# brech1/keaki

Measured on AMD Instinct MI355X. Metric: BN254 G1 scalar-mults/sec on 2^24-point MSM (per GPU), higher is better.
Workload: dtype u32 limbs, 256-bit Montgomery modular integer (9 x 29-bit lazy limbs in the bucket kernel, 8 x 32 elsewhere)

## Files before the change

keaki_amd/csrc/msm.hip.h:

```cpp
#pragma once
#include <type_traits>
#include "bn254_curve.hip.h"
#include "fq29.hip.h"
#include "xyzz29.hip.h"
#include "jac29.hip.h"
#include "xyzz29_g2.hip.h"

namespace bn254 {

typedef uint16_t u16;
typedef u32 v4u_t __attribute__((ext_vector_type(4)));
constexpr u32 DIGIT_NONE = 0xFFFFFFFFu;
#ifndef STAMP
#define STAMP(cond, i) do { } while (0)
#endif

struct MsmShape {
  u32 n;
  u32 c;
  u32 W;
  u32 k;
  u32 stride;
};
KDEV u32 msm_width(const MsmShape& s, u32 w) { return w < s.k ? s.c : s.c - 1; }
KDEV u32 msm_bit_offset(const MsmShape& s, u32 w) { return w < s.k ? w * s.c : s.k * s.c + (w - s.k) * (s.c - 1); }
KDEV u32 msm_nbuckets(const MsmShape& s, u32 w) { u32 wd = msm_width(s, w); return w == s.W - 1 ? (1u << wd) : (1u << (wd - 1)); }
KDEV u32 msm_bucket_base(const MsmShape& s, u32 w) {
  return w <= s.k ? w * (1u << (s.c - 1)) : s.k * (1u << (s.c - 1)) + (w - s.k) * (1u << (s.c - 2));
}
struct MsmPlan {
  MsmShape s;
  size_t nb;
  u32 max_b;
};
inline MsmPlan msm_make_plan(size_t n, int c_target) {
  MsmPlan p;
  u32 W = (254 + c_target - 1) / c_target;
  u32 base = 254 / W, rem = 254 % W;
  p.s.n = (u32)n;
  p.s.W = W;
  p.s.stride = 0;
  if (rem == 0) { p.s.c = base; p.s.k = W; } else { p.s.c = base + 1; p.s.k = rem; }
  size_t nb = 0; u32 mb = 0;
  for (u32 w = 0; w < W; w++) {
    u32 wd = w < p.s.k ? p.s.c : p.s.c - 1;
    u32 b = (w == W - 1) ? (1u << wd) : (1u << (wd - 1));
    nb += b; if (b > mb) mb = b;
  }
  p.nb = nb; p.max_b = mb;
  return p;
}

template <class Emit>
KDEV void msm_for_each_digit_canon(const u32 (&canon)[8], const MsmShape& s, Emit emit) {
  u32 v[8];
#pragma unroll
  for (int j = 0; j < 8; j++) v[j] = canon[j];
  u32 carry = 0;
  for (u32 w = 0; w < s.W; w++) {
    const u32 wd = msm_width(s, w);
    const u32 full = 1u << wd, half = full >> 1;
    u32 coef = (v[0] & (full - 1u)) + carry;
#pragma unroll
    for (int j = 0; j < 7; j++) v[j] = (u32)((((u64)v[j + 1] << 32) | v[j]) >> wd);
    v[7] >>= wd;
    if (w == s.W - 1) {
      if (coef) emit(w, coef - 1u);
    } else if (coef > half) {
      carry = 1;
      if (coef != full) emit(w, (full - coef - 1u) | 0x80000000u);
    } else {
      carry = 0;
      if (coef) emit(w, coef - 1u);
    }
  }
}

template <u32 W> struct StaticPlan {
  static constexpr u32 base = 254 / W, rem = 254 % W;
  static constexpr u32 c = rem ? base + 1 : base, k = rem ? rem : W;
  static constexpr u32 width(u32 w) { return w < k ? c : c - 1; }
  static constexpr u32 offset(u32 w) { return w < k ? w * c : k * c + (w - k) * (c - 1); }
};
template <u32 W>
KDEV void msm_digits_static(const u32 (&v)[8], u32 (&code)[W]) {
  typedef StaticPlan<W> P;
  u32 carry = 0;
#pragma unroll
  for (u32 w = 0; w < W; w++) {
    const u32 off = P::offset(w), wd = P::width(w), j = off >> 5, sh = off & 31;
    const u32 lo = v[j], hi = j + 1 < 8 ? v[j + 1] : 0u;
    const u32 d = (sh + wd <= 32 ? lo >> sh : __builtin_amdgcn_alignbit(hi, lo, sh)) & ((1u << wd) - 1u);
    const u32 full = 1u << wd, half = full >> 1;
    const u32 coef = d + carry;
    if (w == W - 1) {
      code[w] = coef ? coef - 1u : DIGIT_NONE;
    } else {
      const bool neg = coef > half;
      carry = neg ? 1u : 0u;
      code[w] = neg ? (coef != full ? ((full - coef - 1u) | 0x80000000u) : DIGIT_NONE) : (coef ? coef - 1u : DIGIT_NONE);
    }
  }
}

template <class Emit>
KDEV void msm_for_each_digit(const Fr& k, const MsmShape& s, Emit emit) {
  u32 v[8];
  fp_from_mont<FrParams>(v, k);
  msm_for_each_digit_canon(v, s, emit);
}

constexpr u32 T1_THREADS = 1024;
constexpr u32 T1_PER = 3;
constexpr u32 T1_CAP = 36864;
constexpr u32 PART_MAX_BINS = 2048;
constexpr u32 C2_THREADS = 1024;
constexpr u32 C2_CAP = 32768;
constexpr u32 PART_MAX_FINE_SHIFT = 11;
constexpr u32 PART_MAX_FINE = 1u << PART_MAX_FINE_SHIFT;
constexpr u32 SEG_INLINE = 4;
constexpr u32 TE_WPOS = 12, TE_SIGN = 19, TE_FINE = 20, TE_VALID = 0x80000000u;

struct PartShape {
  u32 nbins, lb;
  u32 shift, hb;
  u32 nf;
  u32 tile;
  u32 ntiles;
  u32 te;
  u32 geom;
};
KDEV u32 part_bin(const PartShape& ps, u32 g) { return (g >> ps.shift) & (ps.nbins - 1u); }
KDEV u32 part_fine(const PartShape& ps, u32 g) { return ((g >> (ps.shift + ps.lb)) << ps.shift) | (g & ((1u << ps.shift) - 1u)); }
KDEV u32 part_bucket(const PartShape& ps, u32 bin, u32 f) { return ((f >> ps.shift) << (ps.shift + ps.lb)) | (bin << ps.shift) | (f & ((1u << ps.shift) - 1u)); }
inline bool part_make_shape(size_t n, u32 W, size_t nb, PartShape* ps, int lb_override = -1, int hb_override = -1, int geom_override = -1) {
  u32 lg = 0;
  while (((size_t)1 << lg) < nb) lg++;
  const size_t pairs = n * (size_t)W;
  const u32 lb_max = pairs > ((size_t)C2_CAP << 13) ? 11u : 10u;
  u32 lb = 0;
  while (lb < lb_max && ((size_t)C2_CAP << lb) < pairs) lb++;
  if (lb_override >= 0 && lb_override <= 11) lb = (u32)lb_override;
  if (lb > lg) lb = lg;
  if (lg - lb > PART_MAX_FINE_SHIFT) lb = lg - PART_MAX_FINE_SHIFT;
  if (lb > 11) return false;
  const u32 fb = lg - lb;
  ps->lb = lb; ps->nbins = 1u << lb;
  ps->hb = fb < 3 ? fb : 3u;
  if (hb_override >= 0 && (u32)hb_override <= fb) ps->hb = (u32)hb_override;
  ps->shift = fb - ps->hb;
  ps->nf = 1u << fb;
  u32 tile = W ? T1_CAP / W : T1_THREADS * T1_PER;
  if (tile > T1_THREADS * T1_PER) tile = T1_THREADS * T1_PER;
  if (tile == 0 || W >= (1u << (TE_SIGN - TE_WPOS))) return false;
  ps->tile = tile;
  ps->ntiles = (u32)((n + tile - 1) / tile);
  ps->te = tile * W;
  const u32 mean = ps->te / ps->nbins;
  ps->geom = mean <= 24 ? 0u : mean <= 48 ? 1u : mean <= 100 ? 2u : 3u;
  if (geom_override >= 0) ps->geom = (u32)geom_override;
  return true;
}
inline size_t part_max_chunks(size_t pairs, u32 nbins) { return pairs / C2_CAP + nbins + 1; }

__device__ __forceinline__ void lds_barrier() { asm volatile("s_waitcnt lgkmcnt(0)\n\ts_barrier" ::: "memory"); }

__device__ __forceinline__ u32 lds_exclusive_scan4(u32* a, u32 len, u32* wsum) {
  const u32 t = threadIdx.x, lane = t & 63, wid = t >> 6, nw = blockDim.x >> 6;
  lds_barrier();
  u32 x[4], sum = 0;
#pragma unroll
  for (u32 i = 0; i < 4; i++) { x[i] = 4 * t + i < len ? a[4 * t + i] : 0u; sum += x[i]; }
  u32 v = sum;
#pragma unroll
  for (int o = 1; o < 64; o <<= 1) { u32 y = __shfl_up(v, o, 64); if (lane >= (u32)o) v += y; }
  if (lane == 63) wsum[wid] = v;
  lds_barrier();
  u32 base = 0, tot = 0;
  for (u32 k = 0; k < nw; k++) { u32 sv = wsum[k]; if (k < wid) base += sv; tot += sv; }
  u32 ex = base + v - sum;
#pragma unroll
  for (u32 i = 0; i < 4; i++) { if (4 * t + i < len) a[4 * t + i] = ex; ex += x[i]; }
  lds_barrier();
  return tot;
}

template <u32 WS>
static __global__ void __launch_bounds__(T1_THREADS) k_tile_sort(const Fr* __restrict__ scalars, MsmShape s, PartShape ps, u32* __restrict__ tiles,
                                                                 u16* __restrict__ tstart) {
  __shared__ u32 ent[T1_CAP + 64];
  __shared__ u32 cur[PART_MAX_BINS + 64];
  __shared__ u32 wsum[T1_THREADS / 64];
  constexpr u32 NC = WS ? WS : 1u;
  Fr nxt[T1_PER];
  auto request = [&](u32 tile, u32 tl) {
#pragma unroll
    for (u32 p = 0; p < T1_PER; p++) {
      const u32 li = p * T1_THREADS + tl;
      const size_t i = (size_t)tile * ps.tile + li;
      nxt[p] = scalars[li < ps.tile && i < s.n ? i : (size_t)s.n - 1];
    }
  };
  if (blockIdx.x < ps.ntiles) request(blockIdx.x, threadIdx.x);
  for (u32 tile = blockIdx.x; tile < ps.ntiles; tile += gridDim.x) {
    u32 t = threadIdx.x;
    asm volatile("" : "+v"(t));
    [[maybe_unused]] const u32 sk = (tile - blockIdx.x) / gridDim.x;
    STAMP(blockIdx.x == 100 && t == 0 && sk < 4, 2048 + sk * 16 + 0);
    u32 canon[T1_PER][8];
    bool act[T1_PER];
#pragma unroll
    for (u32 p = 0; p < T1_PER; p++) {
      const u32 li = p * T1_THREADS + t;
      act[p] = li < ps.tile && (size_t)tile * ps.tile + li < s.n;
      fp_from_mont<FrParams>(canon[p], nxt[p]);
    }
    if (tile + gridDim.x < ps.ntiles) request(tile + gridDim.x, t);
    STAMP(blockIdx.x == 100 && t == 0 && sk < 4, 2048 + sk * 16 + 1);
    for (u32 b = t; b < ps.nbins; b += T1_THREADS) cur[b] = 0;
    if (t < 64) cur[PART_MAX_BINS + t] = 0;
    lds_barrier();
    STAMP(blockIdx.x == 100 && t == 0 && sk < 4, 2048 + sk * 16 + 2);
#pragma unroll
    for (u32 p = 0; p < T1_PER; p++) {
      if constexpr (WS != 0) {
        u32 code[NC];
        msm_digits_static<NC>(canon[p], code);
#pragma unroll
        for (u32 w = 0; w < NC; w++) {
          const u32 g = (s.stride ? 0u : msm_bucket_base(s, w)) + (code[w] & 0x7FFFFFFFu);
          atomicAdd(&cur[act[p] && code[w] != DIGIT_NONE ? part_bin(ps, g) : PART_MAX_BINS + (t & 63u)], 1u);
        }
      } else if (act[p]) {
        msm_for_each_digit_canon(canon[p], s, [&](u32 w, u32 cd) {
          const u32 g = (s.stride ? 0u : msm_bucket_base(s, w)) + (cd & 0x7FFFFFFFu);
          atomicAdd(&cur[part_bin(ps, g)], 1u);
        });
      }
    }
    STAMP(blockIdx.x == 100 && t == 0 && sk < 4, 2048 + sk * 16 + 3);
    const u32 m = lds_exclusive_scan4(cur, ps.nbins, wsum);
    u16* ts = tstart + (size_t)tile * (ps.nbins + 1);
    for (u32 b = t; b < ps.nbins; b += T1_THREADS) ts[b] = (u16)cur[b];
    if (t == 0) ts[ps.nbins] = (u16)m;
    lds_barrier();
    STAMP(blockIdx.x == 100 && t == 0 && sk < 4, 2048 + sk * 16 + 4);
#pragma unroll
    for (u32 p = 0; p < T1_PER; p++)
#pragma unroll
      for (u32 j = 0; j < 8; j++) asm volatile("" : "+v"(canon[p][j]));
#pragma unroll
    for (u32 p = 0; p < T1_PER; p++) {
      const u32 li = p * T1_THREADS + t;
      if constexpr (WS != 0) {
        u32 code[NC];
        msm_digits_static<NC>(canon[p], code);
#pragma unroll
        for (u32 w = 0; w < NC; w++) {
          const u32 cd = code[w];
          const bool ok = act[p] && cd != DIGIT_NONE;
          const u32 g = (s.stride ? 0u : msm_bucket_base(s, w)) + (cd & 0x7FFFFFFFu);
          const u32 pos = atomicAdd(&cur[ok ? part_bin(ps, g) : PART_MAX_BINS + (t & 63u)], 1u);
          ent[ok ? pos : T1_CAP + (t & 63u)] = TE_VALID | (part_fine(ps, g) << TE_FINE) | ((cd >> 31) << TE_SIGN) | (w << TE_WPOS) | li;
        }
      } else if (act[p]) {
        msm_for_each_digit_canon(canon[p], s, [&](u32 w, u32 cd) {
          const u32 g = (s.stride ? 0u : msm_bucket_base(s, w)) + (cd & 0x7FFFFFFFu);
          const u32 pos = atomicAdd(&cur[part_bin(ps, g)], 1u);
          ent[pos] = TE_VALID | (part_fine(ps, g) << TE_FINE) | ((cd >> 31) << TE_SIGN) | (w << TE_WPOS) | li;
        });
      }
    }
    STAMP(blockIdx.x == 100 && t == 0 && sk < 4, 2048 + sk * 16 + 5);
    lds_barrier();
    STAMP(blockIdx.x == 100 && t == 0 && sk < 4, 2048 + sk * 16 + 6);
    u32* dst = tiles + (size_t)tile * ps.te;
#pragma unroll 4
    for (u32 q = t; q < m; q += T1_THREADS) dst[q] = ent[q];
    STAMP(blockIdx.x == 100 && t == 0 && sk < 4, 2048 + sk * 16 + 7);
  }
}

static __global__ void __launch_bounds__(1024) k_cell_prefix(const u16* __restrict__ tstart, PartShape ps, uint2* __restrict__ cellmeta,
                                                             u32* __restrict__ bin_total) {
  __shared__ u32 a[4096];
  __shared__ u32 wsum[16];
  const u32 b = blockIdx.x, t = threadIdx.x;
  u32 carry = 0;
  for (u32 base = 0; base < ps.ntiles; base += 4096) {
    u32 st[4], ln[4];
#pragma unroll
    for (u32 k = 0; k < 4; k++) {
      const u32 tile = base + 4 * t + k;
      st[k] = 0; ln[k] = 0;
      if (tile < ps.ntiles) {
        const u16* row = tstart + (size_t)tile * (ps.nbins + 1) + b;
        st[k] = row[0];
        ln[k] = (u32)row[1] - st[k];
      }
      a[4 * t + k] = ln[k];
    }
    const u32 tot = lds_exclusive_scan4(a, 4096, wsum);
#pragma unroll
    for (u32 k = 0; k < 4; k++) {
      const u32 tile = base + 4 * t + k;
      if (tile < ps.ntiles) cellmeta[(size_t)b * ps.ntiles + tile] = make_uint2(carry + a[4 * t + k], st[k] | (ln[k] << 16));
    }
    carry += tot;
    lds_barrier();
  }
  if (t == 0) bin_total[b] = carry;
}
struct BinMeta {
  u32 img_base, chunk_first, nch, total;
};
static __global__ void __launch_bounds__(1024) k_bin_scan(const u32* __restrict__ bin_total, u32 nbins, BinMeta* __restrict__ bins) {
  __shared__ u32 a[2048];
  __shared__ u32 c[2048];
  __shared__ u32 wsum[16];
  const u32 t = threadIdx.x;
  u32 tt[2];
#pragma unroll
  for (u32 k = 0; k < 2; k++) {
    const u32 b = 2 * t + k;
    tt[k] = b < nbins ? bin_total[b] : 0u;
    a[b] = tt[k];
    c[b] = (tt[k] + C2_CAP - 1) / C2_CAP;
  }
  lds_exclusive_scan4(a, 2048, wsum);
  lds_exclusive_scan4(c, 2048, wsum);
#pragma unroll
  for (u32 k = 0; k < 2; k++) {
    const u32 b = 2 * t + k;
    if (b < nbins) bins[b] = {a[b], c[b], (tt[k] + C2_CAP - 1) / C2_CAP, tt[k]};
  }
}

constexpr u32 C2_META = 2048;
KDEV u32 chunk_payload(u32 en, u32 ibase, u32 stride) {
  return (((en >> TE_SIGN) & 1u) << 31) | (ibase + (en & ((1u << TE_WPOS) - 1u)) + ((en >> TE_WPOS) & ((1u << (TE_SIGN - TE_WPOS)) - 1u)) * stride);
}
template <int PHASE>
KDEV void chunk_slow(const u32* __restrict__ tiles, const uint2* __restrict__ cm, const PartShape& ps, u32 stride, u32 c0, u32 lo, u32 hi, u32* hist,
                     u32* pay, u32* sh_next) {
  const u32 grp = threadIdx.x >> 4, l16 = threadIdx.x & 15;
  for (u32 c = c0 + grp; c < ps.ntiles; c += C2_THREADS / 16) {
    const uint2 m = cm[c];
    const u32 len = m.y >> 16;
    if (PHASE == 0 && m.x + len > hi && l16 == 0) atomicMin(sh_next, c);
    if (m.x > hi || (m.x == hi && len)) break;
    const u32 j0 = m.x < lo ? lo - m.x : 0u, j1 = hi - m.x < len ? hi - m.x : len;
    const u32* src = tiles + (size_t)c * ps.te + (m.y & 0xFFFFu);
    for (u32 j = j0 + l16; j < j1; j += 16) {
      const u32 en = src[j];
      const u32 f = (en >> TE_FINE) & (PART_MAX_FINE - 1u);
      if (PHASE == 0) {
        atomicAdd(&hist[f], 1u);
      } else {
        const u32 pos = atomicAdd(&hist[f], 1u);
        pay[pos] = chunk_payload(en, c * ps.tile, stride);
      }
    }
  }
}
template <u32 L, u32 R, u32 Q, bool MASKED = true>
static __global__ void __launch_bounds__(C2_THREADS) k_chunk_sort(const u32* __restrict__ tiles, const uint2* __restrict__ cellmeta,
                                                                  const BinMeta* __restrict__ bins, MsmShape s, PartShape ps, u32 nbuckets_total,
                                                                  u32* __restrict__ sorted, v4u_t* __restrict__ segtab, u32* __restrict__ segoff,
                                                                  u32* __restrict__ bucket_counts) {
  constexpr u32 GROUPS = C2_THREADS / L, CELLS = GROUPS * Q, CAPC = 4 * L * R, NB = 4, QB = Q / NB;
  static_assert(CELLS <= C2_META && Q * R * 4 <= 64 && Q <= 32 && Q % NB == 0 && PART_MAX_FINE == 2 * C2_THREADS, "gather shape");
  __shared__ u32 pay[C2_CAP + 64];
  __shared__ uint2 meta[C2_META];
  __shared__ u32 hist[PART_MAX_FINE + 64];
  __shared__ u32 wsum[C2_THREADS / 64];
  __shared__ u32 sh_next, sh_odd;
  const u32 b = blockIdx.x, t = threadIdx.x, nf = ps.nf;
  const BinMeta bm = bins[b];
  const uint2* cm = cellmeta + (size_t)b * ps.ntiles;
  u32 tot[2] = {0, 0};
  u32 c0 = 0;
  for (u32 f = t; f < PART_MAX_FINE + 64; f += C2_THREADS) hist[f] = 0;
#pragma unroll
  for (u32 i = 0; i < C2_META / C2_THREADS; i++) {
    const u32 ci = t + i * C2_THREADS;
    if (ci < CELLS) meta[ci] = ci < ps.ntiles ? cm[ci] : make_uint2(0xFFFFFFFFu, 0u);
  }
  if (t == 0) { sh_next = ps.ntiles; sh_odd = 0; }
  lds_barrier();
  for (u32 k = 0; k < bm.nch; k++) {
    const u32 lo = k * C2_CAP, hi = bm.total - lo < C2_CAP ? bm.total : lo + C2_CAP;
    u32 tk = t;
    asm volatile("" : "+v"(tk));
    const u32 grp = tk / L, ll = tk % L, dummy = PART_MAX_FINE + (tk & 63u);
    STAMP(b == 100 && t == 0 && k < 8, k * 16 + 0);
    const size_t span = (size_t)(ps.ntiles - c0) * ps.te * 4;
    const __amdgpu_buffer_rsrc_t img = __builtin_amdgcn_make_buffer_rsrc((void*)(tiles + (size_t)c0 * ps.te), 0,
                                                                       span < 0xFFFFFFF0ull ? (u32)span : 0xFFFFFFF0u, 0x00020000);
    auto fetch = [&](u32 tt, u32 q0, u32 (&e)[QB][R][4], u32& longcells, u32& cand, bool& odd) {
      const u32 grp = tt / L, ll = tt % L;
#pragma unroll
      for (u32 qq = 0; qq < QB; qq++) {
        const u32 q = q0 + qq;
        const u32 ci = grp + q * GROUPS;
        const uint2 m = meta[ci];
        const u32 len = m.y >> 16;
        const bool beyond = m.x > hi || (m.x == hi && len);
        if (m.x != 0xFFFFFFFFu && m.x + len > hi && c0 + ci < cand) cand = c0 + ci;
        const u32 j0 = m.x < lo ? lo - m.x : 0u;
        const u32 j1 = beyond ? 0u : (hi - m.x < len ? hi - m.x : len);
        const u32 off = ci * ps.te + (m.y & 0xFFFFu);
#pragma unroll
        for (u32 r = 0; r < R; r++) {
          const u32 j = j0 + 4 * (ll + r * L);
          const v4u_t v = __builtin_amdgcn_raw_buffer_load_b128(img, j < j1 ? (off + j) * 4u : 0xFFFFFFFFu, 0, 0);
#pragma unroll
          for (u32 x = 0; x < 4; x++) e[qq][r][x] = j + x < j1 ? v[x] : 0u;
        }
        if (j1 > j0 + CAPC) longcells |= 1u << q;
        if (q == Q - 1) odd = !beyond && m.x != 0xFFFFFFFFu;
      }
    };
    auto tails = [&](u32 longcells, auto use) {
      while (longcells) {
        const u32 q = __builtin_ctz(longcells);
        longcells &= longcells - 1u;
        const u32 ci = grp + q * GROUPS;
        const uint2 m = meta[ci];
        const u32 len = m.y >> 16;
        const u32 j0 = m.x < lo ? lo - m.x : 0u, j1 = hi - m.x < len ? hi - m.x : len;
        const u32* src = tiles + (size_t)(c0 + ci) * ps.te + (m.y & 0xFFFFu);
        for (u32 j = j0 + CAPC + ll; j < j1; j += L) use(src[j], (c0 + ci) * ps.tile);
      }
    };
    u32 longcells = 0;
    {
      u32 cand = ps.ntiles;
      bool odd = false;
      u32 ea[QB][R][4], eb[QB][R][4];
      u32 th = t;
      asm volatile("" : "+v"(th));
      fetch(th, 0, ea, longcells, cand, odd);
      STAMP(b == 100 && t == 0 && k < 8, k * 16 + 1);
#pragma unroll
      for (u32 h = 0; h < NB; h++) {
        u32 (&cur)[QB][R][4] = h % 2 ? eb : ea;
        if (h + 1 < NB) fetch(th, (h + 1) * QB, h % 2 ? ea : eb, longcells, cand, odd);
#pragma unroll
        for (u32 q = 0; q < QB; q++)
#pragma unroll
          for (u32 r = 0; r < R; r++)
#pragma unroll
            for (u32 x = 0; x < 4; x++) {
              const u32 en = cur[q][r][x];
              if constexpr (MASKED) { if (en) atomicAdd(&hist[(en >> TE_FINE) & (PART_MAX_FINE - 1u)], 1u); }
              else atomicAdd(&hist[en ? (en >> TE_FINE) & (PART_MAX_FINE - 1u) : dummy], 1u);
            }
        __builtin_amdgcn_sched_barrier(0);
      }
      tails(longcells, [&](u32 en, u32) { atomicAdd(&hist[(en >> TE_FINE) & (PART_MAX_FINE - 1u)], 1u); });
      if (ll == 0 && cand < ps.ntiles) atomicMin(&sh_next, cand);
      if (odd) sh_odd = 1;
    }
    STAMP(b == 100 && t == 0 && k < 8, k * 16 + 2);
    lds_barrier();
    STAMP(b == 100 && t == 0 && k < 8, k * 16 + 3);
    const bool slow = sh_odd != 0;
    if (slow) {
      lds_barrier();
      u32 ts = threadIdx.x;
      asm volatile("" : "+v"(ts));
      for (u32 f = ts; f < nf; f += C2_THREADS) hist[f] = 0;
      lds_barrier();
      chunk_slow<0>(tiles, cm, ps, s.stride, c0, lo, hi, hist, pay, &sh_next);
      lds_barrier();
    }
    const u32 c_next = sh_next;
    u32 tm = threadIdx.x;
    asm volatile("" : "+v"(tm));
    uint2 mnext[C2_META / C2_THREADS];
    if (k + 1 < bm.nch) {
#pragma unroll
      for (u32 i = 0; i < C2_META / C2_THREADS; i++) {
        const u32 ci = tm + i * C2_THREADS;
        mnext[i] = ci < CELLS && c_next + ci < ps.ntiles ? cm[c_next + ci] : make_uint2(0xFFFFFFFFu, 0u);
      }
    }
    const u32 x0 = hist[2 * tm], x1 = hist[2 * tm + 1], sum = x0 + x1;
    tot[0] += x0; tot[1] += x1;
    u32 v = sum;
#pragma unroll
    for (int o = 1; o < 64; o <<= 1) { const u32 y = __shfl_up(v, o, 64); if ((tm & 63u) >= (u32)o) v += y; }
    if ((tm & 63u) == 63u) wsum[tm >> 6] = v;
    lds_barrier();
    u32 base = 0;
#pragma unroll
    for (u32 w = 0; w < C2_THREADS / 64; w++) base += w < (tm >> 6) ? wsum[w] : 0u;
    const u32 ex = base + v - sum;
    hist[2 * tm] = ex; hist[2 * tm + 1] = ex + x0;
    {
      const u32 w0 = ex | ((ex + x0) << 16), w1 = (ex + x0) | ((ex + sum) << 16);
      if (k < SEG_INLINE) {
#pragma unroll
        for (u32 i = 0; i < 2; i++) {
          const u32 f = 2 * tm + i, g = part_bucket(ps, b, f);
          if (f < nf && g < nbuckets_total) reinterpret_cast<u32*>(segtab)[(size_t)g * SEG_INLINE + k] = i ? w1 : w0;
        }
      } else if (2 * tm < nf) { u32* so = segoff + (size_t)(bm.chunk_first + k) * nf + 2 * tm; so[0] = w0; so[1] = w1; }
    }
    STAMP(b == 100 && t == 0 && k < 8, k * 16 + 4);
    lds_barrier();
    STAMP(b == 100 && t == 0 && k < 8, k * 16 + 5);
    if (!slow) {
      u32 lc2 = 0, cand = 0;
      bool odd = false;
      u32 ea[QB][R][4], eb[QB][R][4];
      u32 th = t;
      asm volatile("" : "+v"(th));
      fetch(th, 0, ea, lc2, cand, odd);
#pragma unroll
      for (u32 h = 0; h < NB; h++) {
        u32 (&cur)[QB][R][4] = h % 2 ? eb : ea;
        if (h + 1 < NB) fetch(th, (h + 1) * QB, h % 2 ? ea : eb, lc2, cand, odd);
#pragma unroll
        for (u32 q = 0; q < QB; q++) {
          const u32 ibase = (c0 + th / L + (h * QB + q) * GROUPS) * ps.tile;
#pragma unroll
          for (u32 r = 0; r < R; r++)
#pragma unroll
            for (u32 x = 0; x < 4; x++) {
              const u32 en = cur[q][r][x];
              if constexpr (MASKED) {
                if (en) { const u32 pos = atomicAdd(&hist[(en >> TE_FINE) & (PART_MAX_FINE - 1u)], 1u); pay[pos] = chunk_payload(en, ibase, s.stride); }
              } else {
                const u32 pos = atomicAdd(&hist[en ? (en >> TE_FINE) & (PART_MAX_FINE - 1u) : dummy], 1u);
                pay[en ? pos : C2_CAP + (t & 63u)] = chunk_payload(en, ibase, s.stride);
              }
            }
        }
        __builtin_amdgcn_sched_barrier(0);
      }
      tails(lc2, [&](u32 en, u32 ibase) {
        const u32 pos = atomicAdd(&hist[(en >> TE_FINE) & (PART_MAX_FINE - 1u)], 1u);
        pay[pos] = chunk_payload(en, ibase, s.stride);
      });
    } else {
      chunk_slow<1>(tiles, cm, ps, s.stride, c0, lo, hi, hist, pay, &sh_next);
    }
    STAMP(b == 100 && t == 0 && k < 8, k * 16 + 6);
    lds_barrier();
    STAMP(b == 100 && t == 0 && k < 8, k * 16 + 7);
    u32 tw = threadIdx.x;
    asm volatile("" : "+v"(tw));
    u32* dst = sorted + bm.img_base + lo;
#pragma unroll 4
    for (u32 q = tw; q < hi - lo; q += C2_THREADS) dst[q] = pay[q];
    for (u32 f = tw; f < PART_MAX_FINE + 64; f += C2_THREADS) hist[f] = 0;
    if (k + 1 < bm.nch) {
#pragma unroll
      for (u32 i = 0; i < C2_META / C2_THREADS; i++) if (tw + i * C2_THREADS < CELLS) meta[tw + i * C2_THREADS] = mnext[i];
    }
    if (t == 0) { sh_next = ps.ntiles; sh_odd = 0; }
    c0 = c_next;
    STAMP(b == 100 && t == 0 && k < 8, k * 16 + 8);
    lds_barrier();
  }
  u32 te = threadIdx.x;
  asm volatile("" : "+v"(te));
#pragma unroll
  for (u32 i = 0; i < 2; i++) {
    const u32 f = 2 * te + i, g = part_bucket(ps, b, f);
    if (f < nf && g < nbuckets_total) {
      bucket_counts[g] = tot[i];
      for (u32 kk = bm.nch; kk < SEG_INLINE; kk++) reinterpret_cast<u32*>(segtab)[(size_t)g * SEG_INLINE + kk] = 0u;
// ... 761 lines not shown
```

Measured before the change: 1.032 billion.

## Single-pass tile sort: record atomic ranks in packed words and skip second digit pass

For small static window counts, the tile-sort kernel now keeps the rank returned by the counting atomicAdd, packed with the bucket bits into a register word per digit. After the prefix scan it places each entry at start+rank, which removes the second digit extraction and the second round of LDS atomics. If a rank overflows the 9-bit field, a shared flag makes the block fall back to reloading the scalars and running the old two-pass placement. The prefetch of the next tile is moved after the counting pass to ease register pressure, at the cost of more live registers for the packed words.

```diff
diff --git a/keaki_amd/csrc/msm.hip.h b/keaki_amd/csrc/msm.hip.h
--- a/keaki_amd/csrc/msm.hip.h
+++ b/keaki_amd/csrc/msm.hip.h
@@ -185,13 +185,19 @@
   return tot;
 }
 
+constexpr u32 TS_SINGLE_MAX_W = 13;
+constexpr u32 TS_RANK_BITS = 9, TS_SIGN = TS_RANK_BITS, TS_G = TS_SIGN + 1;
+static_assert(TS_G + 11 + PART_MAX_FINE_SHIFT == 32 && (1u << 11) == PART_MAX_BINS && TS_G + 10 == TE_FINE && TS_SIGN + 10 == TE_SIGN,
+              "packed word of the single cut");
 template <u32 WS>
 static __global__ void __launch_bounds__(T1_THREADS) k_tile_sort(const Fr* __restrict__ scalars, MsmShape s, PartShape ps, u32* __restrict__ tiles,
                                                                  u16* __restrict__ tstart) {
   __shared__ u32 ent[T1_CAP + 64];
   __shared__ u32 cur[PART_MAX_BINS + 64];
   __shared__ u32 wsum[T1_THREADS / 64];
+  __shared__ u32 sh_over;
   constexpr u32 NC = WS ? WS : 1u;
+  constexpr bool SINGLE = WS != 0 && WS <= TS_SINGLE_MAX_W;
   Fr nxt[T1_PER];
   auto request = [&](u32 tile, u32 tl) {
 #pragma unroll
@@ -215,15 +221,38 @@
       act[p] = li < ps.tile && (size_t)tile * ps.tile + li < s.n;
       fp_from_mont<FrParams>(canon[p], nxt[p]);
     }
-    if (tile + gridDim.x < ps.ntiles) request(tile + gridDim.x, t);
+    if (!SINGLE && tile + gridDim.x < ps.ntiles) request(tile + gridDim.x, t);
     STAMP(blockIdx.x == 100 && t == 0 && sk < 4, 2048 + sk * 16 + 1);
     for (u32 b = t; b < ps.nbins; b += T1_THREADS) cur[b] = 0;
     if (t < 64) cur[PART_MAX_BINS + t] = 0;
+    if (SINGLE && t == 0) sh_over = 0;
     lds_barrier();
     STAMP(blockIdx.x == 100 && t == 0 && sk < 4, 2048 + sk * 16 + 2);
+    [[maybe_unused]] u32 pk[SINGLE ? T1_PER : 1u][NC];
+    [[maybe_unused]] u32 top = 0;
 #pragma unroll
     for (u32 p = 0; p < T1_PER; p++) {
-      if constexpr (WS != 0) {
+      if constexpr (SINGLE) {
+        u32 code[NC], rank[NC];
+        msm_digits_static<NC>(canon[p], code);
+#pragma unroll
+        for (u32 w = 0; w < NC; w++) {
+          const u32 cd = code[w];
+          const bool ok = act[p] && cd != DIGIT_NONE;
+          const u32 gs = (s.stride ? 0u : msm_bucket_base(s, w)) + cd;
+          const u32 bin = __builtin_amdgcn_ubfe(gs, ps.shift, ps.lb);
+          const u32 one = ok ? 1u : 0u;
+          pk[p][w] = (__builtin_amdgcn_alignbit(gs, gs, 32 - TS_G) & ~((1u << TS_RANK_BITS) - 1u)) | one;
+          rank[w] = atomicAdd(&cur[ok ? bin : PART_MAX_BINS + (t & 63u)], one);
+        }
+#pragma unroll
+        for (u32 w = 0; w < NC; w++) {
+          pk[p][w] += rank[w];
+          asm volatile("" : "+v"(pk[p][w]));
+          top = rank[w] > top ? rank[w] : top;
+        }
+        __builtin_amdgcn_sched_barrier(0);
+      } else if constexpr (WS != 0) {
         u32 code[NC];
         msm_digits_static<NC>(canon[p], code);
 #pragma unroll
@@ -238,6 +267,10 @@
         });
       }
     }
+    if constexpr (SINGLE) {
+      if (top >= (1u << TS_RANK_BITS) - 1u) sh_over = 1;
+      if (tile + gridDim.x < ps.ntiles) request(tile + gridDim.x, t);
+    }
     STAMP(blockIdx.x == 100 && t == 0 && sk < 4, 2048 + sk * 16 + 3);
     const u32 m = lds_exclusive_scan4(cur, ps.nbins, wsum);
     u16* ts = tstart + (size_t)tile * (ps.nbins + 1);
@@ -245,16 +278,11 @@
     if (t == 0) ts[ps.nbins] = (u16)m;
     lds_barrier();
     STAMP(blockIdx.x == 100 && t == 0 && sk < 4, 2048 + sk * 16 + 4);
-#pragma unroll
-    for (u32 p = 0; p < T1_PER; p++)
-#pragma unroll
-      for (u32 j = 0; j < 8; j++) asm volatile("" : "+v"(canon[p][j]));
-#pragma unroll
-    for (u32 p = 0; p < T1_PER; p++) {
+    auto place_cut = [&](u32 p, const u32 (&cn)[8]) {
       const u32 li = p * T1_THREADS + t;
       if constexpr (WS != 0) {
         u32 code[NC];
-        msm_digits_static<NC>(canon[p], code);
+        msm_digits_static<NC>(cn, code);
 #pragma unroll
         for (u32 w = 0; w < NC; w++) {
           const u32 cd = code[w];
@@ -264,12 +292,49 @@
           ent[ok ? pos : T1_CAP + (t & 63u)] = TE_VALID | (part_fine(ps, g) << TE_FINE) | ((cd >> 31) << TE_SIGN) | (w << TE_WPOS) | li;
         }
       } else if (act[p]) {
-        msm_for_each_digit_canon(canon[p], s, [&](u32 w, u32 cd) {
+        msm_for_each_digit_canon(cn, s, [&](u32 w, u32 cd) {
           const u32 g = (s.stride ? 0u : msm_bucket_base(s, w)) + (cd & 0x7FFFFFFFu);
           const u32 pos = atomicAdd(&cur[part_bin(ps, g)], 1u);
           ent[pos] = TE_VALID | (part_fine(ps, g) << TE_FINE) | ((cd >> 31) << TE_SIGN) | (w << TE_WPOS) | li;
         });
       }
+    };
+    if constexpr (SINGLE) {
+      if (__builtin_amdgcn_readfirstlane(sh_over) == 0) {
+        const u32 lowsign = (((1u << ps.shift) - 1u) << TE_FINE) | (1u << TE_SIGN), highmask = ((1u << ps.hb) - 1u) << (TE_FINE + ps.shift);
+        const u32 hrot = (ps.lb + TS_G - TE_FINE) & 31u;
+#pragma unroll
+        for (u32 p = 0; p < T1_PER; p++) {
+          const u32 li = p * T1_THREADS + t;
+          u32 start[NC];
+#pragma unroll
+          for (u32 w = 0; w < NC; w++) start[w] = cur[__builtin_amdgcn_ubfe(pk[p][w], TS_G + ps.shift, ps.lb)];
+#pragma unroll
+          for (u32 w = 0; w < NC; w++) {
+            const u32 k = pk[p][w];
+            const u32 r1 = k & ((1u << TS_RANK_BITS) - 1u);
+            ent[r1 ? start[w] + r1 - 1u : T1_CAP + (t & 63u)] = ((k << (TE_FINE - TS_G)) & lowsign) |
+                                                                (__builtin_amdgcn_alignbit(k, k, hrot) & highmask) | (TE_VALID | (w << TE_WPOS)) | li;
+          }
+        }
+      } else {
+#pragma unroll
+        for (u32 p = 0; p < T1_PER; p++) {
+          const u32 li = p * T1_THREADS + t;
+          const size_t i = (size_t)tile * ps.tile + li;
+          u32 again[8];
+          fp_from_mont<FrParams>(again, scalars[li < ps.tile && i < s.n ? i : (size_t)s.n - 1]);
+          place_cut(p, again);
+          __builtin_amdgcn_sched_barrier(0);
+        }
+      }
+    } else {
+#pragma unroll
+      for (u32 p = 0; p < T1_PER; p++)
+#pragma unroll
+        for (u32 j = 0; j < 8; j++) asm volatile("" : "+v"(canon[p][j]));
+#pragma unroll
+      for (u32 p = 0; p < T1_PER; p++) place_cut(p, canon[p]);
     }
     STAMP(blockIdx.x == 100 && t == 0 && sk < 4, 2048 + sk * 16 + 5);
     lds_barrier();
```

New measurement: 1.032 billion, median of 2. About the same (+0.0%).
